# debbiemarkslab/EVcouplings

Hardware: AMD Instinct MI355X
Metric: plmc L-BFGS iterations/sec (PLM fit, synthetic MSA) (higher is better)
Workload: dtype f32 (forward: f16 hi/lo split couplings on the 2:4 sparse MFMA, f32 accumulation -- in the last iterations of a fit 39-bit fixed-point couplings as five int8 digit planes, exact; backward: 24-bit fixed-point residuals as three int8 digit planes on the int8 MFMA (32-bit / four there), exact int32 acc; 1 GPU; headline: synthetic MSA L=300 q=21 N=50000, theta=0.8, lambda_h=0.01, lambda_J=59.8; parallelism=single GPU

## Files before the change

### evcouplings_amd/csrc/plm_host.cpp

```cpp
#include "../../include/plm_hip.h"
#include "plm_internal.h"

#include <algorithm>
#include <chrono>
#include <cmath>
#include <cstdarg>
#include <cstdio>
#include <cstdlib>
#include <cstring>
#include <string>
#include <vector>

namespace {

thread_local std::string g_err;

int fail(int code, const char *fmt, ...) {
    char buf[512];
    va_list ap;
    va_start(ap, fmt);
    vsnprintf(buf, sizeof buf, fmt, ap);
    va_end(ap);
    g_err = buf;
    return code;
// ... 210 lines not shown
    double dg = cg * gDg;
    for (int k : live) dg += cs[k] * Sg[k] + cy[k] * YDg[k];
    *cg_out = cg;
    *dg_out = dg;
}

struct plm_ctx {
    plm_problem_t prob;
    PlmOptions opt;
    PlmDims d;
    int device = 0;
    hipStream_t st = nullptr;
    plm_exchange_cb exchange = nullptr;
    void *exchange_user = nullptr;
    int8_t *msa_rm = nullptr, *msa_cm = nullptr;
    float *w = nullptr;
    int32_t *counts = nullptr;
    void *Bt = nullptr, *Rt = nullptr;
    int32_t *G = nullptr;
    float *gather = nullptr;
    plm_collective_cb collective = nullptr;
    void *collective_user = nullptr;
    PlmRccl *rccl = nullptr;
    float *xhalo = nullptr, *ghalo = nullptr, *xsend = nullptr, *gsend = nullptr;
    std::vector<int64_t> x_send, x_recv, g_send, g_recv;
    double *fx_part = nullptr, *reg_part = nullptr, *dot_scratch = nullptr, *scal = nullptr;
    uint32_t *maxbits = nullptr;
    int32_t *jexp = nullptr;
    float *x = nullptr, *g = nullptr, *xp = nullptr, *gp = nullptr, *dir = nullptr, *hist = nullptr;
    float *xa = nullptr, *ga = nullptr;
// ... 89 lines not shown
    if (!c->d.sharded) return PLM_OK;
    const int64_t bytes = (int64_t)sizeof(double) * count;
    return ctx_collective(c, PLM_COLL_ALLREDUCE_F64, c->scal + first, c->scal + first, &bytes, &bytes);
}

int group_norms(plm_ctx *c) {
    if (!(c->prob.lambda_group > 0)) return PLM_OK;
    if (!c->pair_n2) PLM_TRY(dalloc(&c->pair_n2, (size_t)std::max<int64_t>(1, c->d.np_own) * 256));
    HIP_TRY(plm_launch_pair_norms(c->d, c->x, c->pair_n2, c->st));
    return PLM_OK;
}
int vp_alloc(plm_ctx *c);
int forward_at_x(plm_ctx *c) {
    const PlmDims &d = c->d;
    PLM_TRY(vp_alloc(c));
    HIP_TRY(plm_launch_forward_store(d, c->msa_rm, c->Bt, c->jexp, c->hj, c->fwd_accurate, c->st));
    HIP_TRY(plm_launch_h64_init(d, c->x, c->h64, c->st));
    HIP_TRY(plm_launch_hpass(d, c->hj, c->msa_rm, c->w, c->h64, 1, 0, c->fwd_accurate, c->Rt, c->fx_part, nullptr, nullptr, nullptr, nullptr, PLM_VP_ALWAYS, c->st));
    return PLM_OK;
}

float *x_rectangles(plm_ctx *c) { return c->x + c->d.nh_pad_l + (size_t)c->d.ntri * PLM_BLOCK_FLOATS(c->d); }

int ctx_eval_enqueue_sharded(plm_ctx *c) {
    const PlmDims &d = c->d;
    PLM_TRY(ctx_collective(c, PLM_COLL_ALLTOALL, x_rectangles(c), c->xhalo, c->x_send.data(), c->x_recv.data()));
    HIP_TRY(plm_launch_maxabs2(c->x + d.nh_pad_l, d.n_local - d.nh_pad_l, c->xhalo,
                               d.nx_halo * (int64_t)PLM_BLOCK_FLOATS(d), c->maxbits, c->jexp, d.jexp_bias, c->st));
    HIP_TRY(plm_launch_expand(d, c->x, c->xhalo, c->jexp, c->Bt, c->fwd_accurate ? 1 : 0, c->st));
    PLM_TRY(forward_at_x(c));
    if (d.nblk_own > 0) HIP_TRY(plm_launch_backward(d, c->msa_cm, c->Rt, c->G, nullptr, c->st));
// ... 72 lines not shown
    return PLM_OK;
}
int vp_stage1(plm_ctx *c) {
    const PlmDims &d = c->d;
    PLM_TRY(vp_counts(c));
    if (d.sharded) {
        PLM_TRY(ctx_collective(c, PLM_COLL_ALLTOALL, x_rectangles(c), c->xhalo, c->x_send.data(), c->x_recv.data()));
        HIP_TRY(plm_launch_maxabs2(c->x + d.nh_pad_l, d.n_local - d.nh_pad_l, c->xhalo,
                                   d.nx_halo * (int64_t)PLM_BLOCK_FLOATS(d), c->maxbits, c->jexp, d.jexp_bias, c->st));
        HIP_TRY(plm_launch_expand(d, c->x, c->xhalo, c->jexp, c->Bt, c->fwd_accurate ? 1 : 0, c->st));
    } else {
        HIP_TRY(plm_launch_maxabs(d, c->x, c->maxbits, c->jexp, c->st));
        HIP_TRY(plm_launch_expand(d, c->x, nullptr, c->jexp, c->Bt, c->fwd_accurate ? 1 : 0, c->st));
    }
    if (c->gemm_ev[0]) HIP_TRY(hipEventRecord(c->gemm_ev[0], c->st));
    HIP_TRY(plm_launch_forward_store(d, c->msa_rm, c->Bt, c->jexp, c->hj, c->fwd_accurate, c->st));
    HIP_TRY(plm_launch_h64_init(d, c->x, c->h64, c->st));
    return PLM_OK;
}
int vp_counts(plm_ctx *c);
int vp_step_and_residuals(plm_ctx *c, bool refresh) {
    const PlmDims &d = c->d;
    PLM_TRY(vp_counts(c));
    const int full = (refresh || c->vp_hess_age < 0) ? 1 : 0;
    HIP_TRY(plm_launch_hpass(d, c->hj, c->msa_rm, c->w, c->h64, 0, full ? 2 : 1, c->fwd_accurate, nullptr, nullptr, c->hpart,
                             c->gpart, c->dpart, nullptr, PLM_VP_ALWAYS, c->st));
    HIP_TRY(plm_launch_hsolve(d, c->hpart, c->gpart, full, c->x, c->h64, c->prob.lambda_h, 1, c->hinv, c->hg2, c->scal + 5, 0.0,
                              0.0, nullptr, 0, c->hcnt, c->dpart, c->st));
    if (full) c->vp_hess_age = 0;
    HIP_TRY(plm_launch_hpass(d, c->hj, c->msa_rm, c->w, c->h64, 1, 1, c->fwd_accurate, c->Rt, c->fx_part, c->hpart, c->gpart,
                             nullptr, nullptr, PLM_VP_ALWAYS, c->st));
// ... 267 lines not shown
    case PLM_ENUMERIC: return "non-finite value in objective";
    case PLM_ECALLBACK: return "exchange callback failed";
    default: return "unknown error";
    }
}

const char *plm_last_error(void) { return g_err.c_str(); }

void plm_ctx_destroy(plm_ctx_t *c) {
    if (!c) return;
    hipSetDevice(c->device);
    for (auto &e : c->gemm_ev)
        if (e) (void)hipEventDestroy(e);
    for (auto &e : c->vp_ev)
        if (e) (void)hipEventDestroy(e);
    void *bufs[] = {c->msa_rm, c->msa_cm, c->w, c->counts, c->Bt, c->Rt, c->G, c->gather, c->fx_part, c->reg_part,
                    c->dot_scratch, c->scal, c->maxbits, c->jexp, c->x, c->g, c->xp, c->gp, c->dir, c->hist,
                    c->canon, c->xhalo, c->ghalo, c->xsend, c->gsend, c->dinv, c->hj, c->hpart, c->gpart, c->dpart, c->hg2, c->hinv, c->h64, c->hcnt, c->vp_flag,
                    c->xa, c->ga, c->pair_n2};
    for (void *b : bufs)
        if (b) hipFree(b);
    if (c->h_scal) hipHostFree(c->h_scal);
    if (c->rccl) {
        hipStreamSynchronize(c->st);
        plm_rccl_destroy(c->rccl);
    }
    delete c;
}

int plm_ctx_create(const plm_problem_t *prob, int device, void *stream, plm_ctx_t **out) {
    if (!prob || !out || !prob->msa) return fail(PLM_EINVAL, "NULL problem / msa / out");
// ... 44 lines not shown
        if (hipMemGetInfo(&free_b, &total_b) == hipSuccess && need > (double)free_b)
            return bail(fail(PLM_ENOMEM, "the problem needs %.1f GB of device memory, %.1f GB are free (of %.1f GB)", need / 1e9,
                             free_b / 1e9, total_b / 1e9));
    }
    if ((rc = dalloc(&c->msa_rm, rm.size())) || (rc = dalloc(&c->msa_cm, cm_size)) ||
        (rc = dalloc(&c->w, (size_t)d.Np)) || (rc = dalloc(&c->counts, (size_t)d.Np)) ||
        (rc = dalloc((char **)&c->Bt, plm_bt_bytes(d))) || (rc = dalloc((char **)&c->Rt, plm_rt_bytes(dmax))) ||
        (rc = dalloc((char **)&c->G, plm_g_bytes(dmax))) || (rc = dalloc(&c->fx_part, (size_t)c->n_fx_part())) ||
        (rc = dalloc(&c->reg_part, (size_t)plm_reg_parts(d))) ||
        (rc = dalloc(&c->dot_scratch, (size_t)4 * PLM_MAX_BASIS * PLM_DOT_BLOCKS)) ||
        (rc = dalloc(&c->scal, (size_t)256)) ||
        (rc = dalloc(&c->maxbits, (size_t)1)) || (rc = dalloc(&c->jexp, (size_t)1)) ||
        (rc = dalloc(&c->x, (size_t)d.n_local)) || (rc = dalloc(&c->g, (size_t)d.n_local)) ||
        (rc = dalloc(&c->canon, (size_t)d.n_canon + (size_t)d.L * d.L)))
        return bail(rc);
    if (d.nshards > 1 && !d.sharded && (rc = dalloc((char **)&c->gather, plm_slab_bytes(d) * d.nshards)))
        return bail(rc);
    if (d.sharded) {
        const size_t blk = PLM_BLOCK_FLOATS(d);
        if ((rc = dalloc(&c->xhalo, (size_t)d.nx_halo * blk)) || (rc = dalloc(&c->gsend, (size_t)d.nx_halo * blk)) ||
            (rc = dalloc(&c->ghalo, (size_t)d.ng_halo * blk)))
            return bail(rc);
        c->x_send.assign(d.nshards, 0); c->x_recv.assign(d.nshards, 0);
        c->g_send.assign(d.nshards, 0); c->g_recv.assign(d.nshards, 0);
        for (int r = 0; r < d.nshards; r++) {
            if (r == d.shard) continue;
            const int64_t mine = plm_half_blocks(d, r), theirs = (int64_t)d.nblk_own * plm_shard_cnt(d, r) - mine;
            c->x_send[r] = c->g_recv[r] = mine * (int64_t)blk * 4;
            c->x_recv[r] = c->g_send[r] = theirs * (int64_t)blk * 4;
        }
    }
    hipError_t e;
    if ((e = hipHostMalloc((void **)&c->h_scal, sizeof(double) * 256)) != hipSuccess)
        return bail(fail(PLM_ENOMEM, "hipHostMalloc failed: %s", hipGetErrorString(e)));
#define CT(expr)                                                                                  \
    if ((e = (expr)) != hipSuccess)                                                               \
        return bail(fail(e == hipErrorOutOfMemory ? PLM_ENOMEM : PLM_EDEVICE, "%s failed: %s", #expr, hipGetErrorString(e)));
    CT(hipMemcpyAsync(c->msa_rm, rm.data(), rm.size(), hipMemcpyHostToDevice, c->st));
    CT(plm_launch_msa_columns(d, c->msa_rm, c->msa_cm, (int)cm_rows, c->st));
    CT(hipMemsetAsync(c->w, 0, sizeof(float) * d.Np, c->st));
    CT(hipMemsetAsync(c->Rt, 0, plm_rt_bytes(dmax), c->st));
    CT(hipMemsetAsync(c->x, 0, sizeof(float) * d.n_local, c->st));
    CT(hipMemsetAsync(c->g, 0, sizeof(float) * d.n_local, c->st));
    CT(hipMemsetAsync(c->scal, 0, sizeof(double) * 256, c->st));
    if (c->gather) CT(hipMemsetAsync(c->gather, 0, plm_slab_bytes(d) * d.nshards, c->st));
    CT(hipStreamSynchronize(c->st));
#undef CT
    *out = c;
    return PLM_OK;
}

int plm_ctx_set_exchange(plm_ctx_t *c, plm_exchange_cb exchange, void *user) {
    if (!c) return fail(PLM_EINVAL, "NULL ctx");
    c->exchange = exchange;
// ... 782 lines not shown
    const bool vp = vp_enabled(c);
    if (vp) PLM_TRY(vp_alloc(c));
    for (int r = 0; r < reps; r++) {
        float ms;
        HIP_TRY(hipEventRecord(ev[0], c->st));
        if (d.sharded) {
            HIP_TRY(plm_launch_maxabs2(c->x + d.nh_pad_l, d.n_local - d.nh_pad_l, c->xhalo,
                                       d.nx_halo * (int64_t)PLM_BLOCK_FLOATS(d), c->maxbits, c->jexp, d.jexp_bias, c->st));
            HIP_TRY(plm_launch_expand(d, c->x, c->xhalo, c->jexp, c->Bt, c->fwd_accurate ? 1 : 0, c->st));
        } else {
            HIP_TRY(plm_launch_maxabs(d, c->x, c->maxbits, c->jexp, c->st));
            HIP_TRY(plm_launch_expand(d, c->x, nullptr, c->jexp, c->Bt, c->fwd_accurate ? 1 : 0, c->st));
        }
        HIP_TRY(hipEventRecord(ev[1], c->st));
        if (vp) {
            HIP_TRY(plm_launch_forward_store(d, c->msa_rm, c->Bt, c->jexp, c->hj, 0, c->st));
            HIP_TRY(hipEventRecord(ev[2], c->st));
            PLM_TRY(vp_step_and_residuals(c, r == 0));
            HIP_TRY(hipEventRecord(ev[5], c->st));
        } else {
            PLM_TRY(forward_at_x(c));
            HIP_TRY(hipEventRecord(ev[2], c->st));
            HIP_TRY(hipEventRecord(ev[5], c->st));
        }
        if (d.nblk_own > 0 || !d.sharded) HIP_TRY(plm_launch_backward(d, c->msa_cm, c->Rt, c->G, nullptr, c->st));
        HIP_TRY(hipEventRecord(ev[3], c->st));
        if (d.sharded) HIP_TRY(plm_launch_pack_g(d, c->G, c->gsend, c->st));
        HIP_TRY(plm_launch_assemble(d, c->G, d.ksplit, d.sharded ? c->ghalo : nullptr, c->x, c->g, c->prob.lambda_h, c->prob.lambda_j,
                                    c->reg_part, vp ? 2 : 0, 0.f, nullptr, 0.f, c->st));
        HIP_TRY(plm_launch_finish_fx(d, c->fx_part, c->n_fx_part(), nullptr, 0, c->reg_part, plm_reg_parts(d),
                                     c->scal, c->st));
// ... 31 lines not shown
            B.n -= 1;
            HIP_TRY(plm_launch_multiaxpy_trial(c->dir, B, C, n, nullptr, m, c->xp, 0.f, c->x, c->st));
            B.n += 1;
        }
        HIP_TRY(hipEventRecord(ev[1], c->st));
        HIP_TRY(hipEventSynchronize(ev[1]));
        float ms;
        HIP_TRY(hipEventElapsedTime(&ms, ev[0], ev[1]));
        acc[PLM_K_LBFGS_VECTOR] = ms;
        HIP_TRY(hipMemsetAsync(c->hist, 0, sizeof(float) * 2 * (size_t)m * n, c->st));
    }
    if (vp && !d.sharded) {
        float ms;
        HIP_TRY(plm_launch_expand(d, c->x, nullptr, c->jexp, c->Bt, 1, c->st));
        HIP_TRY(hipEventRecord(ev[0], c->st));
        for (int r = 0; r < reps; r++) HIP_TRY(plm_launch_forward_store(d, c->msa_rm, c->Bt, c->jexp, c->hj, 1, c->st));
        HIP_TRY(hipEventRecord(ev[1], c->st));
        HIP_TRY(hipEventSynchronize(ev[1]));
        HIP_TRY(hipEventElapsedTime(&ms, ev[0], ev[1]));
        acc[PLM_K_FORWARD_ACCURATE] = ms;
    }
    {
        const int thresh = cluster_threshold(c->prob.theta_id, d.L, d.conv);
        HIP_TRY(hipEventRecord(ev[0], c->st));
        HIP_TRY(plm_launch_reweight(d, c->msa_rm, std::max(1, thresh), c->counts, c->st));
        HIP_TRY(hipEventRecord(ev[1], c->st));
        HIP_TRY(hipEventSynchronize(ev[1]));
        float ms;
        HIP_TRY(hipEventElapsedTime(&ms, ev[0], ev[1]));
        acc[PLM_K_REWEIGHT] = ms * reps;
    }
// ... 389 lines not shown
```

### evcouplings_amd/csrc/plm_internal.h

```cpp
#pragma once
#include <stdint.h>
#include <stddef.h>
#include <hip/hip_runtime.h>

#define PLM_MAX_SHARDS 16
#define PLM_PAD_STATE 127
#define PLM_SEQ_TILE 256
#define PLM_R_EXP 14
#define PLM_BWD_MAXPLANES 4
#define PLM_R_QMAX3 8355000.0f
#define PLM_R_QMAX4 2138000000.0f
#define PLM_BWD_KSTEP 128
#define PLM_BWDW_COLS 9
#define PLM_BWD_ONEHOT_VALUE (-128)

#define PLM_FWD_NG(Q) (((Q) + 2) / 4)
#define PLM_FWD_SPU(Q) (4 * PLM_FWD_NG(Q))
#define PLM_FWD_TILES(Q) (5 * PLM_FWD_NG(Q))

struct PlmDims {
    int N, L, Q;
    int Qc;
    int Np;
    int nb16;
// ... 28 lines not shown
    double theta;
    int sharded;
    int own_lo, own_hi;
    int nblk_own;
    int h_site0;
    int64_t bp_base;
    int64_t np_own;
    int64_t nh_pad_l;
    int64_t n_local;
    int64_t nx_halo;
    int64_t ng_halo;
    int ntri;
    int own_base[PLM_MAX_SHARDS], oth_base[PLM_MAX_SHARDS];
};

struct PlmOptions {
    int bwd_planes = 0;
    int ksplit = 0;
    int fwd_kernel = -1;
    int bwd_kernel = -1;
    int jexp_bias = 0;
    int fwd_mode = -1;
    double acc_factor = 8.0;
    double vp_rel = 1e-4;
    int vp_hess_pos = -1;
    double vp_floor = 2e-7;
    bool debug = false;
    bool debug_vp = false;
};
PlmOptions plm_options_from_env();
// ... 67 lines not shown
static inline __host__ __device__ int64_t plm_pair_index(int i, int j, int L) {
    return (int64_t)i * (2 * L - i - 1) / 2 + (j - i - 1);
}

hipError_t plm_launch_reweight(const PlmDims &d, const int8_t *msa_rm, int thresh, int32_t *counts,
                               hipStream_t st);
hipError_t plm_launch_onehot_rt(const PlmDims &d, const int8_t *msa_rm, const float *w, void *Rt,
                                hipStream_t st);
hipError_t plm_launch_maxabs(const PlmDims &d, const float *x, uint32_t *maxbits, int32_t *jexp,
                             hipStream_t st);
hipError_t plm_launch_expand(const PlmDims &d, const float *x, const float *xhalo, const int32_t *jexp,
                             void *Bt, int exact, hipStream_t st);
hipError_t plm_launch_forward_energy(const PlmDims &d, const int8_t *msa_rm, const void *Bt, const float *x,
                                     const int32_t *jexp, int potentials, int accurate, float *out, hipStream_t st);
hipError_t plm_launch_energy_sum(const PlmDims &d, const float *part, double *out, hipStream_t st);
hipError_t plm_launch_forward_store(const PlmDims &d, const int8_t *msa_rm, const void *Bt, const int32_t *jexp,
                                    float *hj, int exact, hipStream_t st);
int plm_fwd_groups(int q, int exact);
hipError_t plm_launch_hpass(const PlmDims &d, const float *hj, const int8_t *msa_rm, const float *w,
                            const double *h64, int write_rt, int stats, int exact, void *Rt, double *fx_part, float *hpart,
                            double *gpart, double *dpart, const int *state, int cond, hipStream_t st);
#define PLM_VP_HIST 24
#define PLM_VP_MAXBLK 256
struct PlmVpState {
    int done;
    int want_rt;
    int final_skip;
    int passes;
    int cur;
    int pad_;
    double g2_prev;
    double g2_prev2;
// ... 35 lines not shown
hipError_t plm_launch_pack_g(const PlmDims &d, const int32_t *G, float *sendbuf, hipStream_t st);
hipError_t plm_launch_maxabs2(const float *a, int64_t na, const float *b, int64_t nb, uint32_t *maxbits,
                              int32_t *jexp, int jexp_bias, hipStream_t st);
hipError_t plm_launch_finish_fx(const PlmDims &d, const double *fx_part, int n_fx_part,
                                const double *shard_nll, int n_shard_nll, const double *reg_part,
                                int n_reg_part, double *out2 , hipStream_t st);
hipError_t plm_launch_partial_sum(const double *part, int n, double *out, hipStream_t st);
#define PLM_DOT_BLOCKS 1024
hipError_t plm_launch_dots(int npairs, const float *const *a, const float *const *b, int64_t n,
                           double *scratch, double *out, hipStream_t st);
hipError_t plm_launch_lincomb(float *out, float ca, const float *a, float cb, const float *b,
                              int64_t n, hipStream_t st);
hipError_t plm_launch_canon_to_native(const PlmDims &d, const float *xc, float *xn, hipStream_t st);
hipError_t plm_launch_native_to_canon(const PlmDims &d, const float *xn, float *xc, hipStream_t st);
hipError_t plm_launch_fn(const PlmDims &d, const float *jij_canon, float *fn, int a_lo, int g_lo, hipStream_t st);
hipError_t plm_launch_msa_columns(const PlmDims &d, const int8_t *msa_rm, int8_t *msa_cm, int cm_rows, hipStream_t st);
hipError_t plm_launch_compact_gap_blocks(const PlmDims &d, const float *blocks, float *out, hipStream_t st);
hipError_t plm_launch_gap_normalise_pairs(const PlmDims &d, float *fij_canon, double fixed_total, hipStream_t st);
hipError_t plm_launch_align_stats(const int8_t *msa, int n, int L, int gap_state, const int8_t *query, int32_t *seq_gaps,
                                  int32_t *col_gaps, int32_t *ident, hipStream_t st);
size_t plm_bt_bytes(const PlmDims &d);
size_t plm_rt_bytes(const PlmDims &d);
size_t plm_g_bytes(const PlmDims &d);
size_t plm_slab_bytes(const PlmDims &d);
int plm_reg_parts(const PlmDims &d);
bool plm_q_supported(int q);
int plm_q_template(int q);
void plm_pick_tile(int q, int *fm, int *fn);

#define PLM_MAX_BASIS 42
// ... 23 lines not shown
```

### evcouplings_amd/csrc/plm_kernels.hip

```cpp
#include "../../include/plm_hip.h"
#include "plm_internal.h"
#include <math.h>
#include <stdlib.h>
#include <string.h>
#include <mutex>
#include <utility>

typedef _Float16 half8 __attribute__((ext_vector_type(8)));
typedef _Float16 half4 __attribute__((ext_vector_type(4)));
typedef _Float16 half16 __attribute__((ext_vector_type(16)));
typedef float f32x4 __attribute__((ext_vector_type(4)));
typedef int i32x4 __attribute__((ext_vector_type(4)));
typedef unsigned int u32;

#ifndef PLM_DMA_STAGGER_FWD
#define PLM_DMA_STAGGER_FWD 4
#endif
#ifndef PLM_DMA_STAGGER_BWD
#define PLM_DMA_STAGGER_BWD 0
#endif
typedef unsigned long long u64;
#ifndef PLM_ASYNC_A
#define PLM_ASYNC_A 1
#endif
// ... 361 lines not shown
#pragma unroll
    for (int k = 0; k < 16; k++) {
        const int s = s0 + ty * 16 + k, i = i0 + tx;
        int8_t v = (int8_t)PLM_PAD_STATE;
        if (s < d.Np && i < d.Lp32) v = rm[(size_t)s * d.Lp32 + i];
        if (i == ones_row) v = s < d.N ? (int8_t)0 : (int8_t)PLM_PAD_STATE;
        tile[ty * 16 + k][tx] = v;
    }
    __syncthreads();
#pragma unroll
    for (int k = 0; k < 16; k++) {
        const int i = i0 + ty * 16 + k, s = s0 + tx;
        if (i < cm_rows && s < d.Np) cm[(size_t)i * d.Np + s] = tile[tx][ty * 16 + k];
    }
}
hipError_t plm_launch_msa_columns(const PlmDims &d, const int8_t *msa_rm, int8_t *msa_cm, int cm_rows, hipStream_t st) {
    hipLaunchKernelGGL(k_msa_columns, dim3((d.Np + 63) / 64, (cm_rows + 63) / 64), dim3(256), 0, st, d, msa_rm, msa_cm, cm_rows);
    return hipGetLastError();
}

__global__ __launch_bounds__(256) void k_onehot_rt(PlmDims d, const int8_t *__restrict__ msa_rm,
                                                  const float *__restrict__ w, char *__restrict__ Rt) {
    const int s64 = blockIdx.x, b16l = blockIdx.y, b16 = d.b16_lo + b16l;
    for (int idx = threadIdx.x; idx < d.Q * 64; idx += 256) {
        const int a = idx >> 6, lane = idx & 63, kg = lane >> 4, ii = lane & 15;
        const int i = b16 * 16 + ii;
        u32 pw[PLM_BWD_MAXPLANES][4];
        const bool four = d.nplanes == 4;
#pragma unroll
        for (int q4 = 0; q4 < 4; q4++) {
// ... 87 lines not shown
    const int i = b16 * 16 + r;
    const float *__restrict__ xj = x + d.nh_pad_l;
    double s = 0;
    if (!d.gap_mode && i < d.L)
        for (int j = t; j < d.L; j += 64)
            if (j != i) s += (double)load_coupling(d, xj, xhalo, b16, r, a, j >> 4, j & 15, 0);
    for (int o = 32; o > 0; o >>= 1) s += __shfl_down(s, o, 64);
    if (t == 0) {
        cref[((size_t)b16l * 16 + r) * d.Q + a] = (float)s;
        cref64[((size_t)b16l * 16 + r) * d.Q + a] = s;
    }
}
__global__ __launch_bounds__(256) void k_expand(PlmDims d, const float *__restrict__ x,
                                               const float *__restrict__ xhalo,
                                               const int32_t *__restrict__ jexp, _Float16 *__restrict__ Bt) {
    const int NG = PLM_FWD_NG(d.Q), SPU = 4 * NG;
    const int u = blockIdx.x / (2 * NG), ci = blockIdx.x % (2 * NG), b16l = blockIdx.y, b16 = d.b16_lo + b16l;
    const float sc = ldexpf(1.f, *jexp);
    const float *__restrict__ xj = x + d.nh_pad_l;
    _Float16 *tile_hi = Bt + ((size_t)b16l * d.nu * SPU + (size_t)u * SPU + 2 * ci) * (size_t)(2 * d.Q * 512);
    _Float16 *tile_lo = tile_hi + (size_t)(2 * d.Q * 512);
    for (int idx = blockIdx.z * 256 + threadIdx.x; idx < d.Q * 64; idx += gridDim.z * 256) {
        const int a = idx >> 6, lane = idx & 63, gb = lane >> 4, r = lane & 15;
        const int i = b16 * 16 + r;
#pragma unroll
        for (int half = 0; half < 2; half++) {
            half8 hi, lo;
#pragma unroll
            for (int e8 = 0; e8 < 8; e8++) {
                const int ga = 2 * half + (gb >> 1), pp = 2 * (gb & 1) + (e8 >> 2), e = e8 & 3;
                const int gl = 4 * ci + pp, s8 = gl & 7, sg = gl >> 3;
                const int b = 4 * sg + e + 1, j = 32 * u + 8 * ga + s8;
                float v = 0.f;
                if (b < d.Q && i < d.L && j < d.L && i != j) {
                    v = load_coupling(d, xj, xhalo, b16, r, a, j >> 4, j & 15, b);
                    if (!d.gap_mode) v -= load_coupling(d, xj, xhalo, b16, r, a, j >> 4, j & 15, 0);
                    v *= sc;
                }
                const _Float16 h = (_Float16)v;
                hi[e8] = h;
                lo[e8] = (_Float16)(v - (float)h);
            }
            *(half8 *)(tile_hi + (size_t)(half * d.Q + a) * 512 + lane * 8) = hi;
            *(half8 *)(tile_lo + (size_t)(half * d.Q + a) * 512 + lane * 8) = lo;
        }
    }
}

#define PLM_FWDX_PLANES 5
#define PLM_FWDX_SHIFT 23
__global__ __launch_bounds__(256) void k_expand_x(PlmDims d, const float *__restrict__ x,
// ... 34 lines not shown
            w[4][e] = top;
        }
#pragma unroll
        for (int p = 0; p < PLM_FWDX_PLANES; p++)
            *(uint4 *)(t0 + (size_t)p * plane_stride + (size_t)(h16 * d.Q + a) * 1024 + lane * 16) =
                make_uint4(w[p][0], w[p][1], w[p][2], w[p][3]);
    }
}
hipError_t plm_launch_expand(const PlmDims &d, const float *x, const float *xhalo, const int32_t *jexp, void *Bt,
                             int exact, hipStream_t st) {
    if (d.b16_hi <= d.b16_lo) return hipSuccess;
    const int NG = PLM_FWD_NG(d.Q);
    if (exact)
        hipLaunchKernelGGL(k_expand_x, dim3(d.nu * NG, d.b16_hi - d.b16_lo), dim3(256), 0, st, d, x, xhalo, jexp, (char *)Bt);
    else
        hipLaunchKernelGGL(k_expand, dim3(d.nu * 2 * NG, d.b16_hi - d.b16_lo, (d.Q * 64 + 255) / 256), dim3(256), 0, st, d, x, xhalo,
                           jexp, (_Float16 *)Bt);
    hipLaunchKernelGGL(k_fwd_ref, dim3(d.b16_hi - d.b16_lo, 16, d.Q), dim3(64), 0, st, d, x, xhalo,
                       (float *)bt_cref32(d, Bt), (double *)bt_cref64(d, Bt));
    return hipGetLastError();
}

struct FwdArgs {
    const int8_t *msa_rm;
    const char *Bt;
    const float *h;
    const int32_t *jexp;
    float *out;
};
enum { FWD_ENERGY = 1, FWD_POTENTIALS = 2, FWD_STORE = 3 };

template <int QG, int A>
__device__ __forceinline__ void fwd_state(f32x4 (&acc)[2][QG], const half8 &a0, const half8 &a1, int i0, int i1, u32 lb,
                                          half8 (&bh)[3], half8 (&bl)[3], const DmaPlan &dma) {
    constexpr int NP = (2 * QG + 7) / 8;
    if constexpr (A + 2 < QG) {
        bh[(A + 2) % 3] = lds_read_b128<(A + 2) * 1024>(lb);
        bl[(A + 2) % 3] = lds_read_b128<(QG + A + 2) * 1024>(lb);
    }
// ... 23 lines not shown
    extern __shared__ __attribute__((aligned(16))) char smem[];
    constexpr int QG = Q / NSG;
    constexpr int TILE_G = 2 * Q * 1024, TILE = 2 * QG * 1024, NP = (2 * QG + 7) / 8;
    const int tid = threadIdx.x, lane = tid & 63, wave = tid >> 6;
    const int wave_s = __builtin_amdgcn_readfirstlane(wave);
    const int nwork = d.nstiles * (d.b16_hi - d.b16_lo) * NSG, per_xcd = (nwork + 7) >> 3;
    const int wk = (int)(blockIdx.x & 7) * per_xcd + (int)(blockIdx.x >> 3);
    if ((int)(blockIdx.x >> 3) >= per_xcd || wk >= nwork) return;
    const int stile = wk % d.nstiles, sg = (wk / d.nstiles) % NSG, b16l = wk / (d.nstiles * NSG);
    const int tile = b16l * d.nstiles + stile;
    const int a_lo = sg * QG;
    const int b16 = d.b16_lo + b16l;
    const int r = lane & 15, g = lane >> 4;
    const int s_wave = stile * PLM_SEQ_TILE + wave * 32;
    constexpr int NG = PLM_FWD_NG(Q), SPU = 4 * NG;
    const int nsteps = d.nu * SPU;
    const char *bt = A.Bt + (size_t)b16l * nsteps * TILE_G + (size_t)a_lo * 1024;
    const u32 arow0 = (u32)(s_wave + r) * (u32)d.Lp32 + 8 * g, arow1 = arow0 + 16 * (u32)d.Lp32;

    f32x4 acc[2][QG];
#pragma unroll
    for (int a = 0; a < QG; a++) {
        acc[0][a] = (f32x4){0.f, 0.f, 0.f, 0.f};
        acc[1][a] = (f32x4){0.f, 0.f, 0.f, 0.f};
    }
#if PLM_PROBE
    unsigned long long pr_wait = 0;
    const unsigned long long pr_t0 = PROBE_NOW();
#endif
    if (nsteps > 0) {
        const DmaPlan first{bt, smem, wave_s, 2 * QG, (u32)lane * 16, false, nullptr, 0, nullptr, QG, (Q - QG) * 1024};
        dma_issue_all<NP>(first);
    }
    u64 na0 = *(const u64 *)(A.msa_rm + arow0), na1 = *(const u64 *)(A.msa_rm + arow1);
    half8 bh[3], bl[3];
    int t = 0, cur = 0;
    for (int u = 0; u < d.nu; ++u) {
        vm_landed(na0);
        vm_landed(na1);
        const u64 xa0 = na0, xa1 = na1;
        if (u + 1 < d.nu) {
            load_b64_inplace(na0, A.msa_rm, arow0 + 32 * (u + 1));
            load_b64_inplace(na1, A.msa_rm, arow1 + 32 * (u + 1));
        }
        for (int b = 0; b < SPU; ++b, ++t) {
#if PLM_PROBE
            const unsigned long long pa = PROBE_NOW();
#endif
            vm_wait<0>();
            __syncthreads();
#if PLM_PROBE
            pr_wait += PROBE_NOW() - pa;
#endif
            const int nxt = cur ^ 1;
            const DmaPlan dma{bt + (size_t)(t + 1) * TILE_G, smem + nxt * TILE, wave_s, (t + 1 < nsteps) ? 2 * QG : 0,
                              (u32)lane * 16, wave_s >= 4, nullptr, 0, nullptr, QG, (Q - QG) * 1024};
            const u32 lb = lds_addr(smem + cur * TILE + lane * 16);
            half8 a0, a1;
            int i0 = 0, i1 = 0;
            {
                const int ci = b >> 1;
#pragma unroll
                for (int pp = 0; pp < 4; pp++) {
                    const int gl = 4 * ci + pp, s8 = gl & 7, kg = gl >> 3;
                    const u32 x0 = (u32)(xa0 >> (8 * s8)) & 0xffu, x1 = (u32)(xa1 >> (8 * s8)) & 0xffu;
                    ((u32 *)&a0)[pp] = (((x0 - 1u) >> 2) == (u32)kg) ? 0x3C00u : 0u;
                    ((u32 *)&a1)[pp] = (((x1 - 1u) >> 2) == (u32)kg) ? 0x3C00u : 0u;
                    i0 |= (int)(((x0 - 1u) & 3u) << (4 * pp));
                    i1 |= (int)(((x1 - 1u) & 3u) << (4 * pp));
                }
            }
            fwd_kstep<QG>(acc, a0, a1, i0, i1, lb, bh, bl, dma, std::make_integer_sequence<int, QG>{});
            cur = nxt;
        }
    }
#if PLM_PROBE
    if (lane == 0) {
        atomicAdd(&plm_probe_acc[0][0], pr_wait); atomicAdd(&plm_probe_acc[0][3], PROBE_NOW() - pr_t0);
        atomicAdd(&plm_probe_acc[0][5], 1ull);
// ... 257 lines not shown
    constexpr int Q = 21, QG = PLM_FWDW_QG, NSG = Q / QG, NM = PLM_FWDW_NM, SLOT = PLM_FWDW_SLOT;
    constexpr int TILE_G = 2 * Q * 1024, NG = PLM_FWD_NG(Q), SPU = 2 * NG;
    static_assert(NG == 5 && 2 * 2 * QG * 1024 == SLOT, "plm_fwd_asm.inc is generated for 21 states in groups of 7");
    const int tid = threadIdx.x, lane = tid & 63;
    const int wv = __builtin_amdgcn_readfirstlane(tid >> 6);
    const int npair = (d.nstiles + 1) >> 1;
    const int nwork = npair * (d.b16_hi - d.b16_lo) * NSG, per_xcd = (nwork + 7) >> 3;
    const int wk = (int)(blockIdx.x & 7) * per_xcd + (int)(blockIdx.x >> 3);
    if ((int)(blockIdx.x >> 3) >= per_xcd || wk >= nwork) return;
    const int spair = wk % npair, sg = (wk / npair) % NSG, b16l = wk / (npair * NSG);
    const int a_lo = sg * QG;
    const int r = lane & 15, g = lane >> 4;
    const int stile = 2 * spair + (wv >> 1);
    const bool tile_ok = stile < d.nstiles;
    const int s_wave = tile_ok ? stile * PLM_SEQ_TILE + (wv & 1) * 128 : 0;
    const int nsteps = d.nu * SPU;
    const char *bt = A.Bt + (size_t)b16l * nsteps * 2 * TILE_G + (size_t)a_lo * 1024 + wv * 1024;
    const u32 arow = (u32)(s_wave + r) * (u32)d.Lp32 + 8 * g, rstride = 16 * (u32)d.Lp32;

    const u32 l16 = (u32)lane * 16;
    u32 vo[PLM_FWDW_NVMEM];
#pragma unroll
    for (int k = 0; k < PLM_FWDW_NVMEM; k++) {
        const int p = wv + 4 * k, run = p / QG, f = p - run * QG;
        vo[k] = l16 + (u32)((run >> 1) * TILE_G + (run & 1) * Q * 1024 + f * 1024) - (u32)wv * 1024;
    }
    const u32 lw = lds_addr(smem + lane * 16);
    const u32 lw_base = __builtin_amdgcn_readfirstlane(lw - l16);
    const u32 m0t0 = lw_base + wv * 1024;
    const u32 cnt = lw_base + 4 * SLOT;
    if (tid == 0) *(u32 *)(smem + 4 * SLOT) = 0;
    const u32 one = 1, sel = 0x0c0c0200u;
    u32 st, sp;
    asm volatile(PLM_FWDW_ZERO_ASM ::: PLM_FWDW_CLOBBERS);
    for (int i = 0; i < 3; i++) {
        const int stepc = min(i, nsteps - 1);
        asm volatile(PLM_FWDW_ISSUE_ASM
                     :
                     : [tsrc] "s"(bt + (size_t)stepc * 2 * TILE_G), [vo0] "v"(vo[0]), [vo1] "v"(vo[1]), [vo2] "v"(vo[2]),
                       [vo3] "v"(vo[3]), [vo4] "v"(vo[4]), [vo5] "v"(vo[5]), [vo6] "v"(vo[6]), [m0t] "s"(m0t0 + i * SLOT)
                     : "m0", "scc", "memory");
    }
    asm volatile(PLM_FWDW_LOADS_ASM : : [arow] "v"(arow), [rstride] "s"(rstride), [xsrc] "s"(A.msa_rm) : PLM_FWDW_CLOBBERS);
    asm volatile(PLM_FWDW_UPREP_ASM
                 :
                 : [arow] "v"(arow), [rstride] "s"(rstride), [xsrc] "s"(A.msa_rm + 32 * min(1, d.nu - 1)), [sel] "s"(sel)
                 : PLM_FWDW_CLOBBERS);
    vm_wait<0>();
    __syncthreads();
    asm volatile(PLM_FWDW_PRIME_ASM : : [kg] "s"(0), [lbn] "v"(lw) : PLM_FWDW_CLOBBERS);

    int sc = 0;
    u32 tgt = 0;
    const char *tsrc = bt + (size_t)min(3, nsteps - 1) * 2 * TILE_G;
    int step = 0;
#define FWDW_SLICE(WHICH, KG)                                                                                          \
    {                                                                                                                  \
        const int sn = (sc + 1) & 3, snn = (sc + 3) & 3;                                                               \
        asm volatile(WHICH                                                                                             \
                     : [st] "=&s"(st), [sp] "=&s"(sp)                                                                  \
                     : [lb] "v"(lw + sc * SLOT), [lbn] "v"(lw + sn * SLOT), [kg] "s"(KG), [tsrc] "s"(tsrc),          \
                       [vo0] "v"(vo[0]), [vo1] "v"(vo[1]), [vo2] "v"(vo[2]), [vo3] "v"(vo[3]), [vo4] "v"(vo[4]),       \
                       [vo5] "v"(vo[5]), [vo6] "v"(vo[6]), [m0t] "s"(m0t0 + snn * SLOT), [cnt] "v"(cnt),               \
                       [one] "v"(one), [tgt] "s"(tgt)                                                                  \
                     : PLM_FWDW_CLOBBERS);                                                                             \
        sc = sn;                                                                                                       \
        tgt += 4;                                                                                                      \
        tsrc += (step + 4 < nsteps) ? (size_t)2 * TILE_G : 0;               \
        ++step;                                                                                                        \
    }
    for (int u = 0; u < d.nu; ++u) {
#pragma unroll 1
        for (int k = 0; k < NG; ++k) {
            FWDW_SLICE(PLM_FWDW_EVEN_ASM, k)
            if (k == NG - 1)
                asm volatile(PLM_FWDW_UPREP_ASM
                             :
                             : [arow] "v"(arow), [rstride] "s"(rstride),
                               [xsrc] "s"(A.msa_rm + 32 * min(u + 2, d.nu - 1)), [sel] "s"(sel)
                             : PLM_FWDW_CLOBBERS);
            FWDW_SLICE(PLM_FWDW_ODD_ASM, k + 1 < NG ? k + 1 : 0)
        }
    }
#undef FWDW_SLICE
    asm volatile("s_waitcnt vmcnt(0) lgkmcnt(0)\n\ts_nop 15\n\ts_nop 15" ::: "memory");
    if (!tile_ok) return;
    const int je = *A.jexp;
    const double sc64 = ldexp(1.0, -je);
    const double *cref = (const double *)((const float *)(A.Bt + (size_t)d.blk_per_shard * d.nksteps * TILE_G) +
                                          (size_t)d.blk_per_shard * 16 * Q) + ((size_t)b16l * 16 + r) * Q + a_lo;
    float4 *hj = (float4 *)A.out + ((size_t)(b16l * d.nstiles + stile) * 8 + (wv & 1) * 4) * 2 * Q * 64 + (size_t)a_lo * 64 + lane;
    float chi[QG], clo[QG];
#pragma unroll
    for (int a = 0; a < QG; a++) {
        const double c = cref[a];
        chi[a] = (float)c;
        clo[a] = (float)(c - (double)chi[a]);
    }
// ... 39 lines not shown
        if (QQ == 21 && d.fwd_w) return fwdw_launch(d, A, st);                                         \
        return fwd_launch<QQ, FWD_STORE, NP, false>(d, A, st);
    switch (d.Q) {
        FWD_CASE(32, 2, 8)
        FWD_CASE(21, 1, 3)
        FWD_CASE(20, 1, 4)
        FWD_CASE(5, 1, 1)
        FWD_CASE(4, 1, 1)
    default:
        return hipErrorInvalidValue;
    }
#undef FWD_CASE
}
hipError_t plm_launch_forward_energy(const PlmDims &d, const int8_t *msa_rm, const void *Bt, const float *x,
                                     const int32_t *jexp, int potentials, int exact, float *out, hipStream_t st) {
    const FwdArgs A{msa_rm, (const char *)Bt, x, jexp, out};
    return launch_forward_mode(d, A, potentials ? FWD_POTENTIALS : FWD_ENERGY, potentials ? exact : 0, st);
}
hipError_t plm_launch_forward_store(const PlmDims &d, const int8_t *msa_rm, const void *Bt, const int32_t *jexp,
                                    float *hj, int exact, hipStream_t st) {
    const FwdArgs A{msa_rm, (const char *)Bt, nullptr, jexp, hj};
    return launch_forward_mode(d, A, FWD_STORE, exact, st);
}
size_t plm_hj_bytes(const PlmDims &d) { return (size_t)d.nstiles * (d.b16_hi - d.b16_lo) * 8 * 2 * d.Q * 1024; }

#define PLM_HSTATS(Q) ((Q) + (Q) * ((Q) + 1) / 2)
__host__ __device__ constexpr int plm_qc_min(int Q) { return Q == 4 ? 2 : Q == 5 ? 5 : Q == 20 ? 6 : Q == 21 ? 21 : 22; }
#ifndef PLM_HESS_SAMPLE
#define PLM_HESS_SAMPLE 32
#endif
#ifndef PLM_NEWTON_CAP
#define PLM_NEWTON_CAP 3.0
#endif
__device__ __forceinline__ float sum_over_g(float v) {
    unsigned u = __float_as_uint(v);
    auto a = __builtin_amdgcn_permlane32_swap(u, u, false, false);
// ... 2037 lines not shown
```

Measured before the change: 110.5 iterations/s.

## Skip padded half-unit in forward GEMM when site-block count is odd

When the number of 16-site blocks is odd, the forward fp16 path previously processed a full 32-site unit for the last block, doing MFMA work on padding. The Bt expansion layout is now indexed by slices so the tail unit holds only half the slices. The forward kernels run half the steps for that tail, and the wide kernel reads its MSA bytes from a small precomputed tail buffer. This removes wasted coupling expansion and MFMA work for L=300 at the cost of extra indexing logic and an extra buffer and kernel at setup.

After: 110.3 iterations/s. No clear change (-0.2%).

```diff
diff --git a/evcouplings_amd/csrc/plm_host.cpp b/evcouplings_amd/csrc/plm_host.cpp
--- a/evcouplings_amd/csrc/plm_host.cpp
+++ b/evcouplings_amd/csrc/plm_host.cpp
@@ -248,6 +248,7 @@
     plm_exchange_cb exchange = nullptr;
     void *exchange_user = nullptr;
     int8_t *msa_rm = nullptr, *msa_cm = nullptr;
+    int8_t *msa_tail = nullptr;
     float *w = nullptr;
     int32_t *counts = nullptr;
     void *Bt = nullptr, *Rt = nullptr;
@@ -367,7 +368,7 @@
 int forward_at_x(plm_ctx *c) {
     const PlmDims &d = c->d;
     PLM_TRY(vp_alloc(c));
-    HIP_TRY(plm_launch_forward_store(d, c->msa_rm, c->Bt, c->jexp, c->hj, c->fwd_accurate, c->st));
+    HIP_TRY(plm_launch_forward_store(d, c->msa_rm, c->msa_tail, c->Bt, c->jexp, c->hj, c->fwd_accurate, c->st));
     HIP_TRY(plm_launch_h64_init(d, c->x, c->h64, c->st));
     HIP_TRY(plm_launch_hpass(d, c->hj, c->msa_rm, c->w, c->h64, 1, 0, c->fwd_accurate, c->Rt, c->fx_part, nullptr, nullptr, nullptr, nullptr, PLM_VP_ALWAYS, c->st));
     return PLM_OK;
@@ -470,7 +471,7 @@
         HIP_TRY(plm_launch_expand(d, c->x, nullptr, c->jexp, c->Bt, c->fwd_accurate ? 1 : 0, c->st));
     }
     if (c->gemm_ev[0]) HIP_TRY(hipEventRecord(c->gemm_ev[0], c->st));
-    HIP_TRY(plm_launch_forward_store(d, c->msa_rm, c->Bt, c->jexp, c->hj, c->fwd_accurate, c->st));
+    HIP_TRY(plm_launch_forward_store(d, c->msa_rm, c->msa_tail, c->Bt, c->jexp, c->hj, c->fwd_accurate, c->st));
     HIP_TRY(plm_launch_h64_init(d, c->x, c->h64, c->st));
     return PLM_OK;
 }
@@ -768,7 +769,7 @@
         if (e) (void)hipEventDestroy(e);
     for (auto &e : c->vp_ev)
         if (e) (void)hipEventDestroy(e);
-    void *bufs[] = {c->msa_rm, c->msa_cm, c->w, c->counts, c->Bt, c->Rt, c->G, c->gather, c->fx_part, c->reg_part,
+    void *bufs[] = {c->msa_rm, c->msa_tail, c->msa_cm, c->w, c->counts, c->Bt, c->Rt, c->G, c->gather, c->fx_part, c->reg_part,
                     c->dot_scratch, c->scal, c->maxbits, c->jexp, c->x, c->g, c->xp, c->gp, c->dir, c->hist,
                     c->canon, c->xhalo, c->ghalo, c->xsend, c->gsend, c->dinv, c->hj, c->hpart, c->gpart, c->dpart, c->hg2, c->hinv, c->h64, c->hcnt, c->vp_flag,
                     c->xa, c->ga, c->pair_n2};
@@ -843,6 +844,7 @@
         (rc = dalloc(&c->x, (size_t)d.n_local)) || (rc = dalloc(&c->g, (size_t)d.n_local)) ||
         (rc = dalloc(&c->canon, (size_t)d.n_canon + (size_t)d.L * d.L)))
         return bail(rc);
+    if ((d.nb16 & 1) && (rc = dalloc(&c->msa_tail, (size_t)d.Np * 32))) return bail(rc);
     if (d.nshards > 1 && !d.sharded && (rc = dalloc((char **)&c->gather, plm_slab_bytes(d) * d.nshards)))
         return bail(rc);
     if (d.sharded) {
@@ -867,6 +869,7 @@
         return bail(fail(e == hipErrorOutOfMemory ? PLM_ENOMEM : PLM_EDEVICE, "%s failed: %s", #expr, hipGetErrorString(e)));
     CT(hipMemcpyAsync(c->msa_rm, rm.data(), rm.size(), hipMemcpyHostToDevice, c->st));
     CT(plm_launch_msa_columns(d, c->msa_rm, c->msa_cm, (int)cm_rows, c->st));
+    if (c->msa_tail) CT(plm_launch_msa_tail(d, c->msa_rm, c->msa_tail, c->st));
     CT(hipMemsetAsync(c->w, 0, sizeof(float) * d.Np, c->st));
     CT(hipMemsetAsync(c->Rt, 0, plm_rt_bytes(dmax), c->st));
     CT(hipMemsetAsync(c->x, 0, sizeof(float) * d.n_local, c->st));
@@ -1679,7 +1682,7 @@
         }
         HIP_TRY(hipEventRecord(ev[1], c->st));
         if (vp) {
-            HIP_TRY(plm_launch_forward_store(d, c->msa_rm, c->Bt, c->jexp, c->hj, 0, c->st));
+            HIP_TRY(plm_launch_forward_store(d, c->msa_rm, c->msa_tail, c->Bt, c->jexp, c->hj, 0, c->st));
             HIP_TRY(hipEventRecord(ev[2], c->st));
             PLM_TRY(vp_step_and_residuals(c, r == 0));
             HIP_TRY(hipEventRecord(ev[5], c->st));
@@ -1741,7 +1744,7 @@
         float ms;
         HIP_TRY(plm_launch_expand(d, c->x, nullptr, c->jexp, c->Bt, 1, c->st));
         HIP_TRY(hipEventRecord(ev[0], c->st));
-        for (int r = 0; r < reps; r++) HIP_TRY(plm_launch_forward_store(d, c->msa_rm, c->Bt, c->jexp, c->hj, 1, c->st));
+        for (int r = 0; r < reps; r++) HIP_TRY(plm_launch_forward_store(d, c->msa_rm, c->msa_tail, c->Bt, c->jexp, c->hj, 1, c->st));
         HIP_TRY(hipEventRecord(ev[1], c->st));
         HIP_TRY(hipEventSynchronize(ev[1]));
         HIP_TRY(hipEventElapsedTime(&ms, ev[0], ev[1]));
diff --git a/evcouplings_amd/csrc/plm_internal.h b/evcouplings_amd/csrc/plm_internal.h
--- a/evcouplings_amd/csrc/plm_internal.h
+++ b/evcouplings_amd/csrc/plm_internal.h
@@ -66,6 +66,8 @@
     int own_base[PLM_MAX_SHARDS], oth_base[PLM_MAX_SHARDS];
 };
 
+static inline __host__ __device__ int plm_fwd_slices(const PlmDims &d) { return PLM_FWD_NG(d.Q) * d.nb16; }
+
 struct PlmOptions {
     int bwd_planes = 0;
     int ksplit = 0;
@@ -163,8 +165,8 @@
 hipError_t plm_launch_forward_energy(const PlmDims &d, const int8_t *msa_rm, const void *Bt, const float *x,
                                      const int32_t *jexp, int potentials, int accurate, float *out, hipStream_t st);
 hipError_t plm_launch_energy_sum(const PlmDims &d, const float *part, double *out, hipStream_t st);
-hipError_t plm_launch_forward_store(const PlmDims &d, const int8_t *msa_rm, const void *Bt, const int32_t *jexp,
-                                    float *hj, int exact, hipStream_t st);
+hipError_t plm_launch_forward_store(const PlmDims &d, const int8_t *msa_rm, const int8_t *msa_tail, const void *Bt,
+                                    const int32_t *jexp, float *hj, int exact, hipStream_t st);
 int plm_fwd_groups(int q, int exact);
 hipError_t plm_launch_hpass(const PlmDims &d, const float *hj, const int8_t *msa_rm, const float *w,
                             const double *h64, int write_rt, int stats, int exact, void *Rt, double *fx_part, float *hpart,
@@ -230,6 +232,7 @@
 hipError_t plm_launch_canon_to_native(const PlmDims &d, const float *xc, float *xn, hipStream_t st);
 hipError_t plm_launch_native_to_canon(const PlmDims &d, const float *xn, float *xc, hipStream_t st);
 hipError_t plm_launch_fn(const PlmDims &d, const float *jij_canon, float *fn, int a_lo, int g_lo, hipStream_t st);
+hipError_t plm_launch_msa_tail(const PlmDims &d, const int8_t *msa_rm, int8_t *tail, hipStream_t st);
 hipError_t plm_launch_msa_columns(const PlmDims &d, const int8_t *msa_rm, int8_t *msa_cm, int cm_rows, hipStream_t st);
 hipError_t plm_launch_compact_gap_blocks(const PlmDims &d, const float *blocks, float *out, hipStream_t st);
 hipError_t plm_launch_gap_normalise_pairs(const PlmDims &d, float *fij_canon, double fixed_total, hipStream_t st);
diff --git a/evcouplings_amd/csrc/plm_kernels.hip b/evcouplings_amd/csrc/plm_kernels.hip
--- a/evcouplings_amd/csrc/plm_kernels.hip
+++ b/evcouplings_amd/csrc/plm_kernels.hip
@@ -399,6 +399,14 @@
         if (i < cm_rows && s < d.Np) cm[(size_t)i * d.Np + s] = tile[tx][ty * 16 + k];
     }
 }
+__global__ __launch_bounds__(256) void k_msa_tail(PlmDims d, const int8_t *__restrict__ rm, int8_t *__restrict__ tail) {
+    const int idx = blockIdx.x * 256 + threadIdx.x, s = idx >> 3, w = idx & 7;
+    if (s < d.Np) ((u32 *)tail)[idx] = *(const u32 *)(rm + (size_t)s * d.Lp32 + 16 * (d.nb16 - 1) + 4 * (w >> 1));
+}
+hipError_t plm_launch_msa_tail(const PlmDims &d, const int8_t *msa_rm, int8_t *tail, hipStream_t st) {
+    hipLaunchKernelGGL(k_msa_tail, dim3((d.Np * 8 + 255) / 256), dim3(256), 0, st, d, msa_rm, tail);
+    return hipGetLastError();
+}
 hipError_t plm_launch_msa_columns(const PlmDims &d, const int8_t *msa_rm, int8_t *msa_cm, int cm_rows, hipStream_t st) {
     hipLaunchKernelGGL(k_msa_columns, dim3((d.Np + 63) / 64, (cm_rows + 63) / 64), dim3(256), 0, st, d, msa_rm, msa_cm, cm_rows);
     return hipGetLastError();
@@ -516,11 +524,14 @@
 __global__ __launch_bounds__(256) void k_expand(PlmDims d, const float *__restrict__ x,
                                                const float *__restrict__ xhalo,
                                                const int32_t *__restrict__ jexp, _Float16 *__restrict__ Bt) {
-    const int NG = PLM_FWD_NG(d.Q), SPU = 4 * NG;
-    const int u = blockIdx.x / (2 * NG), ci = blockIdx.x % (2 * NG), b16l = blockIdx.y, b16 = d.b16_lo + b16l;
+    const int NG = PLM_FWD_NG(d.Q), nsl = plm_fwd_slices(d);
+    const int sl = blockIdx.x, nfull = d.nb16 >> 1, b16l = blockIdx.y, b16 = d.b16_lo + b16l;
+    const bool tail = sl >= nfull * 2 * NG;
+    const int u = tail ? nfull : sl / (2 * NG), ci = sl - u * 2 * NG;
+    const int sg = tail ? ci : ci >> 1, s0 = tail ? 0 : 4 * (ci & 1), gsites = tail ? 4 : 8;
     const float sc = ldexpf(1.f, *jexp);
     const float *__restrict__ xj = x + d.nh_pad_l;
-    _Float16 *tile_hi = Bt + ((size_t)b16l * d.nu * SPU + (size_t)u * SPU + 2 * ci) * (size_t)(2 * d.Q * 512);
+    _Float16 *tile_hi = Bt + ((size_t)b16l * nsl + sl) * 2 * (size_t)(2 * d.Q * 512);
     _Float16 *tile_lo = tile_hi + (size_t)(2 * d.Q * 512);
     for (int idx = blockIdx.z * 256 + threadIdx.x; idx < d.Q * 64; idx += gridDim.z * 256) {
         const int a = idx >> 6, lane = idx & 63, gb = lane >> 4, r = lane & 15;
@@ -531,12 +542,11 @@
 #pragma unroll
             for (int e8 = 0; e8 < 8; e8++) {
                 const int ga = 2 * half + (gb >> 1), pp = 2 * (gb & 1) + (e8 >> 2), e = e8 & 3;
-                const int gl = 4 * ci + pp, s8 = gl & 7, sg = gl >> 3;
-                const int b = 4 * sg + e + 1, j = 32 * u + 8 * ga + s8;
+                const int b = 4 * sg + e + 1, J = 2 * u + (tail ? 0 : half), jj = (gsites * ga + s0 + pp) & 15, j = 16 * J + jj;
                 float v = 0.f;
                 if (b < d.Q && i < d.L && j < d.L && i != j) {
-                    v = load_coupling(d, xj, xhalo, b16, r, a, j >> 4, j & 15, b);
-                    if (!d.gap_mode) v -= load_coupling(d, xj, xhalo, b16, r, a, j >> 4, j & 15, 0);
+                    v = load_coupling(d, xj, xhalo, b16, r, a, J, jj, b);
+                    if (!d.gap_mode) v -= load_coupling(d, xj, xhalo, b16, r, a, J, jj, 0);
                     v *= sc;
                 }
                 const _Float16 h = (_Float16)v;
@@ -601,7 +611,7 @@
     if (exact)
         hipLaunchKernelGGL(k_expand_x, dim3(d.nu * NG, d.b16_hi - d.b16_lo), dim3(256), 0, st, d, x, xhalo, jexp, (char *)Bt);
     else
-        hipLaunchKernelGGL(k_expand, dim3(d.nu * 2 * NG, d.b16_hi - d.b16_lo, (d.Q * 64 + 255) / 256), dim3(256), 0, st, d, x, xhalo,
+        hipLaunchKernelGGL(k_expand, dim3(plm_fwd_slices(d), d.b16_hi - d.b16_lo, (d.Q * 64 + 255) / 256), dim3(256), 0, st, d, x, xhalo,
                            jexp, (_Float16 *)Bt);
     hipLaunchKernelGGL(k_fwd_ref, dim3(d.b16_hi - d.b16_lo, 16, d.Q), dim3(64), 0, st, d, x, xhalo,
                        (float *)bt_cref32(d, Bt), (double *)bt_cref64(d, Bt));
@@ -610,6 +620,7 @@
 
 struct FwdArgs {
     const int8_t *msa_rm;
+    const int8_t *msa_tail;
     const char *Bt;
     const float *h;
     const int32_t *jexp;
@@ -663,9 +674,11 @@
     const int r = lane & 15, g = lane >> 4;
     const int s_wave = stile * PLM_SEQ_TILE + wave * 32;
     constexpr int NG = PLM_FWD_NG(Q), SPU = 4 * NG;
-    const int nsteps = d.nu * SPU;
+    const int nfull = d.nb16 >> 1, tail_u = (d.nb16 & 1) ? nfull : -1;
+    const int nsteps = 2 * plm_fwd_slices(d);
     const char *bt = A.Bt + (size_t)b16l * nsteps * TILE_G + (size_t)a_lo * 1024;
     const u32 arow0 = (u32)(s_wave + r) * (u32)d.Lp32 + 8 * g, arow1 = arow0 + 16 * (u32)d.Lp32;
+    const u32 tail_back = 8 * (u32)(g - (g >> 1)), tail_shift = 32 * (u32)(g & 1);
 
     f32x4 acc[2][QG];
 #pragma unroll
@@ -681,18 +694,22 @@
         const DmaPlan first{bt, smem, wave_s, 2 * QG, (u32)lane * 16, false, nullptr, 0, nullptr, QG, (Q - QG) * 1024};
         dma_issue_all<NP>(first);
     }
-    u64 na0 = *(const u64 *)(A.msa_rm + arow0), na1 = *(const u64 *)(A.msa_rm + arow1);
+    const u32 back0 = tail_u == 0 ? tail_back : 0u;
+    u64 na0 = *(const u64 *)(A.msa_rm + (arow0 - back0)), na1 = *(const u64 *)(A.msa_rm + (arow1 - back0));
     half8 bh[3], bl[3];
     int t = 0, cur = 0;
     for (int u = 0; u < d.nu; ++u) {
         vm_landed(na0);
         vm_landed(na1);
-        const u64 xa0 = na0, xa1 = na1;
+        const bool tail = u == tail_u;
+        const u64 xa0 = tail ? na0 >> tail_shift : na0, xa1 = tail ? na1 >> tail_shift : na1;
         if (u + 1 < d.nu) {
-            load_b64_inplace(na0, A.msa_rm, arow0 + 32 * (u + 1));
-            load_b64_inplace(na1, A.msa_rm, arow1 + 32 * (u + 1));
-        }
-        for (int b = 0; b < SPU; ++b, ++t) {
+            const u32 back = u + 1 == tail_u ? tail_back : 0u;
+            load_b64_inplace(na0, A.msa_rm, arow0 + 32 * (u + 1) - back);
+            load_b64_inplace(na1, A.msa_rm, arow1 + 32 * (u + 1) - back);
+        }
+        const int nb = tail ? SPU / 2 : SPU;
+        for (int b = 0; b < nb; ++b, ++t) {
 #if PLM_PROBE
             const unsigned long long pa = PROBE_NOW();
 #endif
@@ -709,9 +726,10 @@
             int i0 = 0, i1 = 0;
             {
                 const int ci = b >> 1;
+                const int s8_0 = tail ? 0 : 4 * (ci & 1), kg = tail ? ci : ci >> 1;
 #pragma unroll
                 for (int pp = 0; pp < 4; pp++) {
-                    const int gl = 4 * ci + pp, s8 = gl & 7, kg = gl >> 3;
+                    const int s8 = s8_0 + pp;
                     const u32 x0 = (u32)(xa0 >> (8 * s8)) & 0xffu, x1 = (u32)(xa1 >> (8 * s8)) & 0xffu;
                     ((u32 *)&a0)[pp] = (((x0 - 1u) >> 2) == (u32)kg) ? 0x3C00u : 0u;
                     ((u32 *)&a1)[pp] = (((x1 - 1u) >> 2) == (u32)kg) ? 0x3C00u : 0u;
@@ -999,9 +1017,11 @@
     const int stile = 2 * spair + (wv >> 1);
     const bool tile_ok = stile < d.nstiles;
     const int s_wave = tile_ok ? stile * PLM_SEQ_TILE + (wv & 1) * 128 : 0;
-    const int nsteps = d.nu * SPU;
+    const int nfull = d.nb16 >> 1, has_tail = d.nb16 & 1;
+    const int nsteps = plm_fwd_slices(d);
     const char *bt = A.Bt + (size_t)b16l * nsteps * 2 * TILE_G + (size_t)a_lo * 1024 + wv * 1024;
     const u32 arow = (u32)(s_wave + r) * (u32)d.Lp32 + 8 * g, rstride = 16 * (u32)d.Lp32;
+    const u32 arow_t = (u32)(s_wave + r) * 32u + 8 * g, rstride_t = 16 * 32u;
 
     const u32 l16 = (u32)lane * 16;
     u32 vo[PLM_FWDW_NVMEM];
@@ -1026,11 +1046,22 @@
                        [vo3] "v"(vo[3]), [vo4] "v"(vo[4]), [vo5] "v"(vo[5]), [vo6] "v"(vo[6]), [m0t] "s"(m0t0 + i * SLOT)
                      : "m0", "scc", "memory");
     }
-    asm volatile(PLM_FWDW_LOADS_ASM : : [arow] "v"(arow), [rstride] "s"(rstride), [xsrc] "s"(A.msa_rm) : PLM_FWDW_CLOBBERS);
-    asm volatile(PLM_FWDW_UPREP_ASM
-                 :
-                 : [arow] "v"(arow), [rstride] "s"(rstride), [xsrc] "s"(A.msa_rm + 32 * min(1, d.nu - 1)), [sel] "s"(sel)
-                 : PLM_FWDW_CLOBBERS);
+#define FWDW_XSRC(UN)                                                                                                  \
+    const int un_ = min((UN), d.nu - 1);                                                                               \
+    const bool ut_ = has_tail && un_ == nfull;                                                                         \
+    const int8_t *xsrc_ = ut_ ? A.msa_tail : A.msa_rm + 32 * un_;                                                      \
+    const u32 arow_ = ut_ ? arow_t : arow, rstride_ = ut_ ? rstride_t : rstride;
+    {
+        FWDW_XSRC(0)
+        asm volatile(PLM_FWDW_LOADS_ASM : : [arow] "v"(arow_), [rstride] "s"(rstride_), [xsrc] "s"(xsrc_) : PLM_FWDW_CLOBBERS);
+    }
+    {
+        FWDW_XSRC(1)
+        asm volatile(PLM_FWDW_UPREP_ASM
+                     :
+                     : [arow] "v"(arow_), [rstride] "s"(rstride_), [xsrc] "s"(xsrc_), [sel] "s"(sel)
+                     : PLM_FWDW_CLOBBERS);
+    }
     vm_wait<0>();
     __syncthreads();
     asm volatile(PLM_FWDW_PRIME_ASM : : [kg] "s"(0), [lbn] "v"(lw) : PLM_FWDW_CLOBBERS);
@@ -1054,19 +1085,28 @@
         tsrc += (step + 4 < nsteps) ? (size_t)2 * TILE_G : 0;               \
         ++step;                                                                                                        \
     }
-    for (int u = 0; u < d.nu; ++u) {
+    for (int u = 0; u < nfull; ++u) {
 #pragma unroll 1
         for (int k = 0; k < NG; ++k) {
             FWDW_SLICE(PLM_FWDW_EVEN_ASM, k)
-            if (k == NG - 1)
+            if (k == NG - 1) {
+                FWDW_XSRC(u + 2)
                 asm volatile(PLM_FWDW_UPREP_ASM
                              :
-                             : [arow] "v"(arow), [rstride] "s"(rstride),
-                               [xsrc] "s"(A.msa_rm + 32 * min(u + 2, d.nu - 1)), [sel] "s"(sel)
+                             : [arow] "v"(arow_), [rstride] "s"(rstride_), [xsrc] "s"(xsrc_), [sel] "s"(sel)
                              : PLM_FWDW_CLOBBERS);
+            }
             FWDW_SLICE(PLM_FWDW_ODD_ASM, k + 1 < NG ? k + 1 : 0)
         }
     }
+    if (has_tail) {
+#pragma unroll 1
+        for (int k = 0; k < NG; k += 2) {
+            FWDW_SLICE(PLM_FWDW_EVEN_ASM, k + 1 < NG ? k + 1 : 0)
+            if (k + 1 < NG) FWDW_SLICE(PLM_FWDW_ODD_ASM, k + 2 < NG ? k + 2 : 0)
+        }
+    }
+#undef FWDW_XSRC
 #undef FWDW_SLICE
     asm volatile("s_waitcnt vmcnt(0) lgkmcnt(0)\n\ts_nop 15\n\ts_nop 15" ::: "memory");
     if (!tile_ok) return;
@@ -1136,12 +1176,13 @@
 }
 hipError_t plm_launch_forward_energy(const PlmDims &d, const int8_t *msa_rm, const void *Bt, const float *x,
                                      const int32_t *jexp, int potentials, int exact, float *out, hipStream_t st) {
-    const FwdArgs A{msa_rm, (const char *)Bt, x, jexp, out};
+    const FwdArgs A{msa_rm, nullptr, (const char *)Bt, x, jexp, out};
     return launch_forward_mode(d, A, potentials ? FWD_POTENTIALS : FWD_ENERGY, potentials ? exact : 0, st);
 }
-hipError_t plm_launch_forward_store(const PlmDims &d, const int8_t *msa_rm, const void *Bt, const int32_t *jexp,
-                                    float *hj, int exact, hipStream_t st) {
-    const FwdArgs A{msa_rm, (const char *)Bt, nullptr, jexp, hj};
+hipError_t plm_launch_forward_store(const PlmDims &d, const int8_t *msa_rm, const int8_t *msa_tail, const void *Bt,
+                                    const int32_t *jexp, float *hj, int exact, hipStream_t st) {
+    if (!exact && d.Q == 21 && d.fwd_w && (d.nb16 & 1) && !msa_tail) return hipErrorInvalidValue;
+    const FwdArgs A{msa_rm, msa_tail, (const char *)Bt, nullptr, jexp, hj};
     return launch_forward_mode(d, A, FWD_STORE, exact, st);
 }
 size_t plm_hj_bytes(const PlmDims &d) { return (size_t)d.nstiles * (d.b16_hi - d.b16_lo) * 8 * 2 * d.Q * 1024; }
```
